# turlando/flac-py

Measured on AMD Instinct MI355X. Metric: PCM samples/sec encode-analysis, 4608-blk/16-bit mono, 1/2/4/8 MI355X, higher is better.
Workload: dtype i16 in; f64 autocorrelation/Levinson; i32 predictors; 1 GPU; 1e6 synthetic mono 4608-sample int16 blocks, -l 12 -q 5 -r 0,5; units_per_gpu=1000000, units_total=1000000, block=4608, sample_bits=16, max_lpc_order=12, qlp_precision=5, mode=reference, parallelism=dp1 (block shards), open_eighths=0, lpc_pruning=on: candidates proven to lose skipped (sign bound, partial-sum tiers)

## Files before the change

### flac-py_amd/csrc/flacmi_host.cpp

```cpp
#include <dlfcn.h>
#include <hip/hip_runtime.h>

#include <algorithm>
#include <atomic>
#include <cerrno>
#include <chrono>
#include <cmath>
#include <cstdarg>
#include <cstdio>
#include <cstdlib>
#include <cstring>
#include <map>
#include <mutex>
#include <string>
#include <vector>

#include "../../include/flacmi.h"
#include "flacmi_kernels.h"
#include "pymath.h"
#include "device_common.h"

using namespace flacmi;

static double (*volatile libm_cos)(double) = cos;
// ... 94 lines not shown
    return w;
}

struct DevBuf {
    void* p = nullptr;
    size_t bytes = 0;
};

struct flacmi_ctx {
    int device = 0;
    hipStream_t stream = nullptr;
    double* d_log2thr = nullptr;
    int32_t* d_sintab = nullptr;
    std::map<int, double*> windows;
    std::map<int, std::pair<int, int>> window_one;
    DevBuf rec, retry, h_samples, h_meta, h_params, h_residual, h_acf, h_fs, h_ls, h_recs;
    uint16_t* d_crc = nullptr;
    DevBuf scan, h_offsets, h_status, h_frames, dec, slow;
    DevBuf h_subkind;
    DevBuf h_side, h_choice;
    DevBuf idx, sd_data, sd_table, sd_meta, sd_rows, sd_pcm;
    int64_t frames_bytes = 0;
    static constexpr int kRing = 64;
    static constexpr int kMaxChunks = 8;
    hipEvent_t ev[kRing][3 + 2 * kMaxChunks] = {};
    int nchunks[kRing] = {};
    hipEvent_t lpc_done[kMaxChunks] = {};
    int ncalls = 0;
    struct EncState* enc = nullptr;
};
static void enc_free(struct EncState* es);
// ... 117 lines not shown
    if ((e = hipMemcpy(ctx->d_sintab, g_sintab.data(), sizeof(int32_t) * 4096, hipMemcpyHostToDevice)) != hipSuccess)
        return bad(e, "hipMemcpy");
    const std::vector<uint16_t> crc = crc16_tables();
    if ((e = hipMalloc(&ctx->d_crc, sizeof(uint16_t) * crc.size())) != hipSuccess) return bad(e, "hipMalloc");
    if ((e = hipMemcpy(ctx->d_crc, crc.data(), sizeof(uint16_t) * crc.size(), hipMemcpyHostToDevice)) != hipSuccess)
        return bad(e, "hipMemcpy");
    return ctx;
}

void flacmi_destroy(flacmi_ctx* ctx) {
    if (!ctx) return;
    (void)hipSetDevice(ctx->device);
    (void)hipDeviceSynchronize();
    enc_free(ctx->enc);
    for (auto& kv : ctx->windows) (void)hipFree(kv.second);
    for (DevBuf* b : {&ctx->idx, &ctx->sd_data, &ctx->sd_table, &ctx->sd_meta, &ctx->sd_rows, &ctx->sd_pcm, &ctx->slow, &ctx->dec, &ctx->rec, &ctx->retry, &ctx->h_samples, &ctx->h_meta, &ctx->h_params, &ctx->h_residual, &ctx->h_acf,
                      &ctx->h_fs, &ctx->h_ls, &ctx->h_recs, &ctx->scan, &ctx->h_offsets, &ctx->h_status,
                      &ctx->h_frames, &ctx->h_subkind, &ctx->h_side, &ctx->h_choice})
        if (b->p) (void)hipFree(b->p);
    if (ctx->d_log2thr) (void)hipFree(ctx->d_log2thr);
    if (ctx->d_sintab) (void)hipFree(ctx->d_sintab);
    if (ctx->d_crc) (void)hipFree(ctx->d_crc);
    for (auto& slot : ctx->ev)
        for (auto& ev : slot)
            if (ev) (void)hipEventDestroy(ev);
    if (ctx->stream) (void)hipStreamDestroy(ctx->stream);
    for (auto& ev : ctx->lpc_done)
        if (ev) (void)hipEventDestroy(ev);
    delete ctx;
}

// ... 143 lines not shown
}

constexpr int64_t kOverlapMinUnits = 16384;
static int overlap_mode() { return knob(kKnobOverlap); }

static int analyze_device_impl(flacmi_ctx* ctx, const flacmi_batch* b, const flacmi_params* p,
                               const flacmi_outputs* o, hipStream_t s, bool allow_overlap = true) {
    if (int rc = set_device(ctx)) return rc;
    const bool lpc = p->mode == FLACMI_MODE_REFERENCE || p->mode == FLACMI_MODE_LPC_ONLY;
    const int L = lpc ? p->max_lpc_order : 0;
    const int rec_words = FLACMI_LPC_REC_WORDS(L);
    if (lpc) {
        if (int rc = ensure_buf(ctx->rec, sizeof(int32_t) * (size_t)rec_words * (size_t)(b->n_units > 0 ? b->n_units : 1)))
            return rc;
    }
    constexpr int64_t kSubWords = 64 * 16;
    if (int rc = ensure_buf(ctx->retry, sizeof(int64_t) * (size_t)(kSubWords + 2 * b->n_units + 68))) return rc;
    struct Cls {
        int64_t unit0, count;
        int n;
    } cls[2];
    int ncls = 0;
    const int64_t nfull = b->n_units - b->n_tail_units;
    if (b->n_tail_units == 0 || b->tail_len == b->block_len) {
        cls[ncls++] = {0, b->n_units, b->block_len};
    } else {
        if (nfull > 0) cls[ncls++] = {0, nfull, b->block_len};
        cls[ncls++] = {nfull, b->n_tail_units, b->tail_len};
    }
    if (o->acf && !lpc)
// ... 23 lines not shown
                ch[nch++] = {cls[c].unit0, whole, cls[c].n};
                ch[nch++] = {cls[c].unit0 + whole, rest, cls[c].n};
                overlap = true;
                continue;
            }
        }
        int64_t k = overlap && ov > 1 ? cls[c].count / kOverlapMinUnits : 1;
        const int left = flacmi_ctx::kMaxChunks - nch - (ncls - 1 - c);
        k = k < 1 ? 1 : k > want ? want : k;
        k = k > left ? left : k;
        for (int64_t i = 0; i < k; ++i) {
            const int64_t u0 = cls[c].count * i / k, u1 = cls[c].count * (i + 1) / k;
            ch[nch++] = {cls[c].unit0 + u0, u1 - u0, cls[c].n};
        }
    }
    auto lpc_args = [&](const Chunk& k, LpcArgs& a) -> int {
        a = LpcArgs{};
        a.samples = b->samples;
        a.stride = b->unit_stride;
        a.unit0 = k.unit0;
        a.count = k.count;
        a.sample_bytes = b->sample_bytes;
        a.n = k.n;
        a.L = L;
        a.q = p->qlp_precision;
        a.lpc_sign = (p->reserved[1] & FLACMI_FLAG_LPC_SIGN) != 0;
        if (int rc = get_window(ctx, k.n, (double**)&a.window, &a.fuse_lo, &a.fuse_hi)) return rc;
        if (b->sample_bits > 26) a.fuse_lo = a.fuse_hi = 0;
        a.log2thr = ctx->d_log2thr;
        a.rec = (int32_t*)ctx->rec.p + k.unit0 * rec_words;
        a.rec_words = rec_words;
        a.acf = o->acf ? o->acf + k.unit0 * 33 : nullptr;
        return 0;
    };
    auto launch_resid_chunk = [&](const Chunk& k, hipStream_t st) -> hipError_t {
        ResidArgs a{};
        a.samples = b->samples;
        a.stride = b->unit_stride;
        a.unit0 = k.unit0;
        a.count = k.count;
        a.sample_bytes = b->sample_bytes;
        a.n = k.n;
        a.L = L;
        a.mode = p->mode;
        a.rmin = p->rice_min;
        a.rmax = p->rice_max;
        a.rec = lpc ? (const int32_t*)ctx->rec.p + k.unit0 * rec_words : nullptr;
        a.rice_order = p->mode == FLACMI_MODE_RICE_ONLY ? p->reserved[0] : 0;
        a.rec_words = rec_words;
        a.log2thr = ctx->d_log2thr;
        a.meta = o->meta + k.unit0;
        a.rice_params = o->rice_params + k.unit0 * o->params_stride;
        a.params_stride = o->params_stride;
        a.residual = (char*)o->residual + (size_t)k.unit0 * o->residual_stride * o->residual_bytes;
        a.residual_stride = o->residual_stride;
        a.fixed_sums = o->fixed_sums ? o->fixed_sums + k.unit0 * 5 : nullptr;
        a.lpc_sums = o->lpc_sums ? o->lpc_sums + k.unit0 * 32 : nullptr;
        a.stop_after = debug_stop();
        a.mfma = use_mfma();
        int64_t* const rb = (int64_t*)ctx->retry.p;
        a.retry_sub = (unsigned long long*)rb;
        a.retry_count = (unsigned long long*)(rb + kSubWords);
        a.retry_list = rb + kSubWords + 2;
        a.retry2_count = (unsigned long long*)(rb + kSubWords + 2 + b->n_units + 64);
        a.retry2_list = rb + kSubWords + 4 + b->n_units + 64;
        a.sample_bits = b->sample_bits;
        a.stream = use_stream();
        a.prune = p->mode == FLACMI_MODE_REFERENCE && !o->lpc_sums &&
                  !(p->reserved[1] & (FLACMI_FLAG_ALL_CANDIDATES | FLACMI_FLAG_LPC_SIGN)) && prune_allowed();
        a.sign_bound = !(p->reserved[1] & FLACMI_FLAG_TIERS_ONLY) && sign_bound_allowed();
        const bool wide = needs_wide(k.n, b->sample_bits, L, p->qlp_precision, p->mode);
        int path = (wide || o->residual_bytes == 8) ? 2 : (b->sample_bytes == 2 && p->qlp_precision <= 16) ? 0 : 1;
        if (path == 2 && o->residual_bytes == 4 && split_ok(b->sample_bits, L, p->qlp_precision)) path = 3;
        return launch_resid(a, path, o->residual_bytes, st);
    };
    const int slot = ctx->ncalls % flacmi_ctx::kRing;
    hipEvent_t* ev = ctx->ev[slot];
    hipStream_t side = nullptr;
    if (overlap && !allow_overlap) overlap = false;
    if (overlap) {
        if (int rc = enc_streams(ctx)) return rc;
        side = enc_side(ctx);
        if (side == s) overlap = false;
    }
    ctx->nchunks[slot] = overlap ? nch : 0;
    HIP_TRY(hipEventRecord(ev[0], s));
    if (overlap) {
        HIP_TRY(hipStreamWaitEvent(side, ev[0], 0));
// ... 1456 lines not shown
```

### flac-py_amd/csrc/flacmi_kernels.h

```cpp
#pragma once
#include <hip/hip_runtime.h>
#include <stdint.h>

#include "../../include/flacmi.h"

namespace flacmi {

constexpr int kWindowPad = 80;

struct LpcArgs {
    const void* samples;
    int64_t stride;
    int64_t unit0, count;
    int32_t sample_bytes;
    int32_t n, L, q;
    const double* window;
    const double* log2thr;
    int32_t* rec;
    int32_t rec_words;
    int32_t lpc_sign;
    double* acf;
    int32_t fuse_lo, fuse_hi;
};

struct ResidArgs {
    const void* samples;
    int64_t stride;
    int64_t unit0, count;
    int32_t sample_bytes;
    int32_t n, L, mode;
    int32_t rmin, rmax;
    int32_t rice_order;
    const int32_t* rec;
    int32_t rec_words;
    const double* log2thr;
    flacmi_unit_meta* meta;
    int32_t* rice_params;
// ... 3 lines not shown
    int64_t* fixed_sums;
    int64_t* lpc_sums;
    int32_t stop_after;
    int32_t mfma;
    unsigned long long* retry_count;
    int64_t* retry_list;
    unsigned long long* retry2_count;
    int64_t* retry2_list;
    unsigned long long* retry_sub;
    int64_t retry_sub_cap;
    int32_t sample_bits;
    int32_t stream;
    int32_t prune;
    int32_t persist;
    int32_t sign_bound;
};
#define FLACMI_STATUS_RETRY 0x7e

struct StereoChoice {
    int32_t code;
    int32_t status;
    int64_t unit[2];
};

struct FrameArgs {
    const void* samples;
    int64_t stride;
    int32_t sample_bytes;
    int32_t block_len, tail_len;
    int64_t n_units, n_tail_units;
// ... 115 lines not shown
};

ResidLaunch resid_launch_config(int n, int rmax_eff, int residual_bytes);
constexpr int kMaxFinestParts = 4096;

enum Knob { kKnobOverlap = 0, kKnobMf8Grid, kKnobStreamGeneric, kKnobDecodeGeneric, kKnobPackGeneric, kKnobDecodeLpc, kKnobCount };
int knob(Knob k);

hipError_t launch_lpc(const LpcArgs& a, hipStream_t s);
int64_t lpc_units_per_round(const LpcArgs& a);
hipError_t launch_poison_lds(hipStream_t s);
hipError_t launch_export(const int64_t* off, const int32_t* st, int64_t nf, int64_t* h_off, int32_t* h_st,
                         hipStream_t s);
hipError_t launch_lpc_from_acf(const LpcArgs& a, hipStream_t s);
hipError_t launch_resid(const ResidArgs& a, int path, int residual_bytes, hipStream_t s);
hipError_t launch_expand_records(const int32_t* rec, int32_t rec_words, int32_t L, int64_t count,
                                 int32_t* out, hipStream_t s);
hipError_t launch_synth(void* dst, int32_t sample_bytes, int32_t bits, int64_t stride,
                        int64_t first_unit, int64_t n_units, int32_t len, uint64_t seed,
                        const int32_t* sintab, int32_t open8, hipStream_t s);
hipError_t launch_stats(const flacmi_unit_meta* meta, int64_t n_units, int32_t block_len,
                        int32_t tail_len, int64_t n_tail_units, int64_t* stats, hipStream_t s);

hipError_t launch_stereo_rows(const void* lr, int32_t sample_bytes, int64_t lr_stride, int64_t n_frames,
                              int32_t block_len, int32_t tail_len, int32_t has_tail, void* mid, int64_t mid_stride,
                              int32_t* side, int64_t side_stride, hipStream_t s);
hipError_t launch_stereo_choose(const FrameArgs& a, hipStream_t s);

hipError_t launch_frame_sizes(const FrameArgs& a, int64_t* bsum, hipStream_t s);
int64_t frame_scan_blocks(int64_t n_frames);
// ... 11 lines not shown
```

### flac-py_amd/csrc/k_lpc.hip

```cpp
#include <type_traits>

#include <map>
#include <mutex>
#include <utility>

#include "device_common.h"

namespace flacmi {


template <int LMAX>
__device__ __forceinline__ void write_quant(int32_t* rec, int L, int p, const int32_t* q, int nq,
                                            int shift) {
    rec[2 + p - 1] = shift;
    int32_t* c = rec + 2 + L + (p * (p - 1)) / 2;
#pragma unroll
    for (int j = 0; j < LMAX; ++j)
        if (j < p) c[j] = j < nq ? q[j] : 0;
}

template <int LMAX>
__device__ __forceinline__ void lpc_finish(const double (&acc)[LMAX + 1], const LpcArgs& a, int32_t* __restrict__ rec) {
    const int L = a.L, q = a.q;
    const pym::PowTables PT{c_log_hdr, c_log_tab, c_exp_hdr, c_exp_tab};
    double c[LMAX + 1];
    c[0] = 1.0;
#pragma unroll
    for (int j = 1; j <= LMAX; ++j) c[j] = 0.0;
    double err = acc[0];
    int lst = ST_OK, lsite = 0, qst = ST_OK, qsite = 0;
    uint32_t negmask = 0;
    const double qmax = (double)((1LL << (q - 1)) - 1);
    const double qmin = -(double)(1LL << (q - 1));
    const uint64_t sign = a.lpc_sign ? 1ull << 63 : 0;
    static_for<LMAX>([&](auto K_) {
        constexpr int k = K_;
        if (k < L && lst == ST_OK) {
            double lam = 0.0;
#pragma unroll
            for (int j = 0; j <= k; ++j) lam = lam - c[j] * acc[k + 1 - j];
            if (err == 0.0) {
                lst = ST_ZERODIV;
                lsite = FLACMI_SITE_LEVINSON_DIV;
            } else {
                lam = lam / err;
#pragma unroll
                for (int nn = 0; nn <= (k + 1) / 2; ++nn) {
                    const double tmp = c[k + 1 - nn] + lam * c[nn];
                    c[nn] = c[nn] + lam * c[k + 1 - nn];
                    c[k + 1 - nn] = tmp;
                }
// ... 2 lines not shown
                if (pst) {
                    lst = ST_OVERFLOW;
                    lsite = FLACMI_SITE_LEVINSON_POW;
                } else {
                    err = err * (1.0 - l2);
                }
            }
            if (lst == ST_OK && qst == ST_OK) {
                const int p = k + 1;
                double cm = __builtin_fabs(c[1]);
#pragma unroll
                for (int j = 2; j <= LMAX; ++j)
                    if (j <= p && __builtin_fabs(c[j]) > cm) cm = __builtin_fabs(c[j]);
                int32_t* __restrict__ cq = rec + 2 + L + (p * (p - 1)) / 2;
                int shift = 0;
                if (!(cm > 0.0)) {
                    qst = ST_ASSERT;
                    qsite = FLACMI_SITE_QUANT_CMAX;
                } else if (__builtin_isinf(cm)) {
                    qst = ST_OVERFLOW;
                    qsite = FLACMI_SITE_QUANT_LOG2;
                } else {
                    shift = q - pym::py_floor_log2(cm, a.log2thr) - 2;
                    if (shift > 15) shift = 15;
                    if (shift < -16) {
                        qst = ST_ASSERT;
                        qsite = FLACMI_SITE_QUANT_SHIFT;
                    } else {
                        const bool neg = shift < 0;
                        const double scale = pym::as_double(((uint64_t)(1023 + (neg ? -shift : shift)) << 52) | sign);
// ... 1 lines not shown
#pragma unroll
                        for (int j = 1; j <= LMAX; ++j) {
                            if (j <= p && qst == ST_OK) {
                                e = e + c[j] * scale;
                                if (__builtin_isinf(e)) {
                                    qst = ST_OVERFLOW;
                                    qsite = FLACMI_SITE_QUANT_ROUND_INF;
                                } else if (__builtin_isnan(e)) {
                                    qst = ST_VALUE;
                                    qsite = FLACMI_SITE_QUANT_ROUND_NAN;
                                } else {
                                    const double r = __builtin_rint(e);
                                    const double qq = r < qmin ? qmin : (r > qmax ? qmax : r);
                                    e = e - qq;
                                    cq[j - 1] = (int32_t)qq;
                                }
                            }
                        }
                        if (qst == ST_OK) {
                            if (neg) {
                                negmask |= 1u << k;
                                shift = 0;
#pragma unroll
                                for (int j = 0; j < LMAX; ++j)
                                    if (j < p) cq[j] = 0;
                            }
                            rec[2 + p - 1] = shift;
                        }
                    }
                }
            }
        }
    });
    int st = lst != ST_OK ? lst : qst;
    int site = lst != ST_OK ? lsite : qsite;
    if (st == ST_OK && L == 0) {
        st = ST_VALUE;
        site = FLACMI_SITE_LPC_EMPTY;
    }
    rec[0] = st | (site << 16);
    rec[1] = (int32_t)negmask;
}

constexpr int lpc_waves(int lmax, int sample_bytes = 4) { return lmax <= 12 ? 3 : sample_bytes == 4 ? 2 : 1; }

template <int LMAX, typename SampleT, bool ACF_IN = false>
__global__ __launch_bounds__(256) __attribute__((amdgpu_waves_per_eu(lpc_waves(LMAX, (int)sizeof(SampleT))))) void k_lpc(LpcArgs a) {
    const int64_t gid = (int64_t)blockIdx.x * 256 + threadIdx.x;
    if (gid >= a.count) return;
    const int64_t u = a.unit0 + gid;
    const SampleT* __restrict__ x = (const SampleT*)a.samples + u * a.stride;
    int32_t* __restrict__ rec = a.rec + gid * a.rec_words;
    const int n = a.n, L = a.L;

    constexpr int S = ((LMAX + 1 + 7) / 8) * 8;
    double acc[LMAX + 1];
// ... 144 lines not shown
                    }
                }
            }
        }
#pragma unroll
        for (int w = 0; w < W; ++w) cur[w] = nxt[w];
    }
    }
    if (a.acf) {
        double* o = a.acf + gid * 33;
#pragma unroll
        for (int l = 0; l < 33; ++l) o[l] = (l <= LMAX && l <= L) ? acc[l < LMAX ? l : LMAX] : 0.0;
    }
    }

    lpc_finish<LMAX>(acc, a, rec);
}


template <int LMAX>
__global__ __launch_bounds__(256) __attribute__((amdgpu_waves_per_eu(LMAX <= 12 ? 4 : 1))) void k_lpc_tile(LpcArgs a) {
    __shared__ __align__(16) uint4 tiles[4 * 512];
    const int lane = threadIdx.x & 63, wid = threadIdx.x >> 6;
    const int64_t wave0 = (int64_t)blockIdx.x * 256 + wid * 64;
    if (wave0 >= a.count) return;
    const int64_t gid = wave0 + lane;
    const int n = a.n, L = a.L;
    int32_t* __restrict__ rec = a.rec + gid * a.rec_words;
    constexpr int S = ((LMAX + 1 + 7) / 8) * 8;
    static_assert(32 % S == 0, "ring length divides a half tile");
    static_assert(64 <= kWindowPad, "the last tile's window reads stay inside the window's zero pad");
// ... 86 lines not shown
    };
    int t1 = (a.fuse_lo + LMAX + 63) >> 6;
    if (a.fuse_lo + LMAX <= 0) t1 = 0;
    int t2 = min(a.fuse_hi, M) >> 6;
    if (t2 > ntile) t2 = ntile;
    if (t1 > t2) t1 = t2;
    if (ntile > 0) issue(0);
    for (int tI = 0; tI < t1; ++tI) tile_body(tI, T0{});
    for (int tI = t1; tI < t2; ++tI) tile_body(tI, T1{});
    for (int tI = t2; tI < ntile; ++tI) tile_body(tI, T0{});
    if (a.acf) {
        double* o = a.acf + gid * 33;
#pragma unroll
        for (int l = 0; l < 33; ++l) o[l] = (l <= LMAX && l <= L) ? acc[l < LMAX ? l : LMAX] : 0.0;
    }
    lpc_finish<LMAX>(acc, a, rec);
}


static bool lpc_tile_enabled() {
    static const bool on = [] {
        const char* e = getenv("FLACMI_LPC_TILE");
        return !(e && e[0] == '0');
    }();
    return on;
}

template <int LMAX>
static hipError_t launch_lpc_T(const LpcArgs& a, hipStream_t s) {
    const dim3 grid((unsigned)((a.count + 255) / 256));
    if constexpr (LMAX <= 12) {
        const int64_t full = a.count & ~(int64_t)63;
        if (a.sample_bytes == 2 && lpc_tile_enabled() && a.stride % 8 == 0 && a.stride >= 8 && full > 0) {
            LpcArgs t = a;
            t.count = full;
            hipLaunchKernelGGL((k_lpc_tile<LMAX>), dim3((unsigned)((full + 255) / 256)), dim3(256), 0, s, t);
            if (full == a.count) return hipGetLastError();
            LpcArgs r = a;
            r.unit0 += full;
            r.count = a.count - full;
            r.rec += full * a.rec_words;
            if (r.acf) r.acf += full * 33;
            hipLaunchKernelGGL((k_lpc<LMAX, int16_t>), dim3((unsigned)((r.count + 255) / 256)), dim3(256), 0, s, r);
            return hipGetLastError();
        }
    }
    if (a.sample_bytes == 2)
        hipLaunchKernelGGL((k_lpc<LMAX, int16_t>), grid, dim3(256), 0, s, a);
    else
        hipLaunchKernelGGL((k_lpc<LMAX, int32_t>), grid, dim3(256), 0, s, a);
    return hipGetLastError();
}

hipError_t launch_lpc_from_acf(const LpcArgs& a, hipStream_t s) {
    if (a.count <= 0) return hipSuccess;
    hipLaunchKernelGGL((k_lpc<32, int32_t, true>), dim3((unsigned)((a.count + 255) / 256)), dim3(256), 0, s, a);
// ... 42 lines not shown
```

### flac-py_amd/csrc/k_stream.hip

```cpp
#include <type_traits>

#include "device_common.h"

namespace flacmi {

namespace {

typedef _Float16 h8 __attribute__((ext_vector_type(8)));
typedef float f4 __attribute__((ext_vector_type(4)));
typedef _Float16 h2 __attribute__((ext_vector_type(2)));
typedef unsigned short us2 __attribute__((ext_vector_type(2)));

#ifndef FLACMI_STREAM_CPT
#define FLACMI_STREAM_CPT 5
#endif
constexpr int kSCPT = FLACMI_STREAM_CPT;
#ifndef FLACMI_RICE_DEDUP
#define FLACMI_RICE_DEDUP 1
#endif
#ifndef FLACMI_SAD16
#define FLACMI_SAD16 1
#endif
__host__ __device__ constexpr int stream_threads(int n) {
    const int nch = n / 8;
    const int nt = 64 * ((nch + 64 * kSCPT - 1) / (64 * kSCPT));
    return nt < 64 ? 64 : nt;
}
constexpr int kSHP = 16;
constexpr uint32_t kMagicBits = 0x4B400000u;
constexpr int kCoefLimit = 127;
constexpr int kRiceOrders = 8;

struct SLds {
    int xs, pk, rec, red, red2, red0, pks, total;
};

__host__ __device__ inline SLds stream_lds(int n, int nw, int tap_words, int P, int RS) {
    auto up = [](int b) { return (b + 15) & ~15; };
    auto mx = [](int x, int y) { return x > y ? x : y; };
    SLds l;
    int o = 0;
    l.xs = o;   o = up(o + 2 * (kSHP + n));
    l.pk = l.rec = o; o = up(o + mx(2 * P * RS, 4 * mx(tap_words, 1)));
    l.red = l.red2 = o; o = up(o + mx(8 * nw * 16, 8 * (nw + 1) * kRiceOrders));
    l.red0 = o; o = up(o + 4 * nw);
    l.pks = o;  o = up(o + 4 * P);
    l.total = o;
    return l;
}

__host__ __device__ constexpr int tap_table_words(int NG) { return NG > 0 ? 40 * NG + 1 : 0; }
__device__ __forceinline__ uint32_t f16_of_int(int v) {
    return (uint32_t)__builtin_bit_cast(unsigned short, (_Float16)(float)v);
}

constexpr uint32_t f16_bits(int v) {
    if (v == 0) return 0;
    const uint32_t sgn = v < 0 ? 0x8000u : 0u;
    const int m = v < 0 ? -v : v;
    int e = 0;
    while ((m >> (e + 1)) != 0) ++e;
    return sgn | (uint32_t)((e + 15) << 10) | (uint32_t)((m << (10 - e)) & 0x3ff);
}
constexpr int fixed_tap(int p, int j) {
    if (j == 0) return -1;
    if (j < 0 || j > p) return 0;
    int c = 1;
    for (int t = 0; t < j; ++t) c = c * (p - t) / (t + 1);
    return (j & 1) ? c : -c;
// ... 157 lines not shown
template <int NG, bool R05, int NFIX, bool LIST, typename Args>
__device__ __forceinline__ void stream_unit(const Args& a, const int64_t gid, unsigned char* smem) {
    const int tid = LIST ? (int)opaque((uint32_t)threadIdx.x) : (int)threadIdx.x, NT = NFIX ? stream_threads(NFIX) : (int)blockDim.x, lane = tid & 63, nw = NT >> 6;
#if FLACMI_STREAM_STAMPS
    uint64_t stamp[8];
    const uint64_t rt0 = __builtin_amdgcn_s_memrealtime();
    stamp[0] = __builtin_amdgcn_s_memtime();
#define STAMP(k) (stamp[k] = __builtin_amdgcn_s_memtime())
#else
#define STAMP(k) ((void)0)
#endif
    const int wid = __builtin_amdgcn_readfirstlane(tid >> 6);
    const int n = NFIX ? NFIX : a.n, L = NG > 0 ? (NFIX ? 4 * NG : a.L) : 0;
    const int nch = n >> 3, nblk = n >> 6;
    const int rw = NG > 0 ? (NFIX ? 2 + L + (L * (L + 1)) / 2 : a.rec_words) : 0;
    int rmax_eff = -1;
    for (int o = a.rmin; o <= a.rmax; ++o)
        if (n % (1 << o) == 0) rmax_eff = o;
    const int Pmax = 1 << rmax_eff;
    constexpr int RS = kRiceOrders;
    const SLds lay = stream_lds(n, nw, tap_table_words(NG), Pmax, RS);
    uint16_t* xs = reinterpret_cast<uint16_t*>(smem + lay.xs) + kSHP;
    int32_t* recl = reinterpret_cast<int32_t*>(smem + lay.rec);
    uint32_t* red0 = reinterpret_cast<uint32_t*>(smem + lay.red0);
    unsigned long long* red2 = reinterpret_cast<unsigned long long*>(smem + lay.red2);
    uint32_t* pks = reinterpret_cast<uint32_t*>(smem + lay.pks);
    uint16_t* pkw = reinterpret_cast<uint16_t*>(smem + lay.pk);
    flacmi_unit_meta* meta = a.meta + gid;
    MetaVals mv{};

    uint4 fixb;
    {
        const uint4* src = reinterpret_cast<const uint4*>((const int16_t*)a.samples + (a.unit0 + gid) * a.stride);
        uint4 q[kSCPT];
#pragma unroll
        for (int j = 0; j < kSCPT; ++j) {
#if FLACMI_NT_LOAD
            typedef unsigned int v4u __attribute__((ext_vector_type(4)));
            const v4u t = __builtin_nontemporal_load(reinterpret_cast<const v4u*>(src) + min(tid + j * NT, nch - 1));
            q[j] = uint4{t.x, t.y, t.z, t.w};
#else
            q[j] = src[min(tid + j * NT, nch - 1)];
#endif
        }
        fixb = reinterpret_cast<const uint4*>(kFixB.w)[lane];
        constexpr int kTW = tap_table_words(NG), kTJ = NG > 0 ? (kTW + 63) / 64 : 0;
        int32_t tv[kTJ > 0 ? kTJ : 1][2];
        if constexpr (NG > 0) {
            const int32_t* r = a.rec + gid * rw;
#pragma unroll
            for (int j = 0; j < kTJ; ++j) {
                if (j > 0 && j * NT >= kTW) break;
                const int gw = tid + j * NT, p = gw / 10 + 1, w = gw - 10 * (p - 1);
                const int pc = p < L ? p : L, base = 2 + L + (pc * (pc - 1)) / 2;
                tv[j][0] = r[w == 8 ? 1 + pc : min(max(base + 15 - 2 * w, 0), rw - 1)];
                tv[j][1] = r[min(max(base + 14 - 2 * w, 0), rw - 1)];
            }
        }
        if (tid < kSHP) xs[tid - kSHP] = 0x8000u;
        if (tid < Pmax) pks[tid] = a.stop_after == 10 ? (uint32_t)n * 40u : 0u;
#if FLACMI_SAD16
        const uint32_t k8000 = opaque(0x80008000u);
#else
        const uint32_t k8000 = opaque(0x8000u);
#endif
        uint32_t sumx = 0;
#pragma unroll
        for (int j = 0; j < kSCPT; ++j) {
            const int v = tid + j * NT;
            if (v < nch) {
                const uint4 y{q[j].x ^ 0x80008000u, q[j].y ^ 0x80008000u, q[j].z ^ 0x80008000u, q[j].w ^ 0x80008000u};
// ... 3 lines not shown
                for (int e = 0; e < 4; ++e) {
#if FLACMI_SAD16
                    sumx = __builtin_amdgcn_sad_u16(yd[e], k8000, sumx);
#else
                    sumx = sad32(yd[e] & 0xffffu, k8000, sumx);
                    sumx = sad32(yd[e] >> 16, k8000, sumx);
#endif
                }
            }
        }
        if constexpr (NG > 0) {
            uint32_t* tt = reinterpret_cast<uint32_t*>(recl);
#pragma unroll
            for (int j = 0; j < kTJ; ++j) {
                if (j > 0 && j * NT >= kTW) break;
                const int gw = tid + j * NT, p = gw / 10 + 1, w = gw - 10 * (p - 1);
                if (gw < kTW) {
                    auto tap = [&](int i, int32_t c) -> uint32_t {
                        if (p > L || i < 0 || i > p) return 0u;
                        return f16_of_int(i == 0 ? -(1 << c) : c);
                    };
                    tt[gw] = tap(16 - 2 * w, tv[j][0]) | tap(15 - 2 * w, tv[j][1]) << 16;
                }
            }
        }
        const uint32_t sx = wave_sum_u32(sumx);
        if (lane == 0) red0[wid] = sx;
    }
    STAMP(1);
    __syncthreads();
    STAMP(2);
    uint32_t negmask = 0;
    const int32_t* __restrict__ grec = NG > 0 ? a.rec + gid * rw : nullptr;
    if constexpr (NG > 0) {
        const int st = grec[0];
        if (st != 0) {
            if (wid == 0) {
                mv.status = st & 0xffff;
                mv.site = st >> 16;
                store_meta(meta, lane, mv, 0);
            }
            return;
        }
        negmask = (uint32_t)grec[1];
    }

    const bool prune = NG > 0 && a.prune && !LIST;
    unsigned long long* red64 = reinterpret_cast<unsigned long long*>(smem + lay.red);
    auto lane_total = [&]() __attribute__((always_inline)) -> uint64_t {
        uint64_t t = 0;
        int g = -1, o4l = 0;
        if (lane >= 1 && lane <= 4) {
            g = 0;
            o4l = lane - 1;
        } else if (NG > 0 && lane >= 16 && lane < 16 + 4 * NG) {
            g = 1 + ((lane - 16) >> 2);
            o4l = (lane - 16) & 3;
        }
        if (g >= 0) {
// ... 2 lines not shown
        } else if (lane == 0) {
#pragma unroll 1
            for (int w2 = 0; w2 < nw; ++w2) t += red0[w2];
        }
        return t;
    };
    uint64_t tj = 0;
    bool pruned = false;
    {
        const int col = lane & 15, kb = lane >> 4, o4 = col >> 2, rho = col & 3;
        h8 B[NG + 1];
        int shg[NG + 1];
        const uint32_t* tt = reinterpret_cast<const uint32_t*>(recl);
        const int k0 = 4 + 4 * kb - rho;
        const uint32_t alb = 16u * (uint32_t)(k0 & 1);
        bool outside = false;
#pragma unroll
        for (int g = 0; g <= NG; ++g) {
            int sh = 0;
            if (g == 0) {
                B[0] = __builtin_bit_cast(h8, fixb);
            } else {
                const int p = 4 * (g - 1) + o4 + 1, wb = 10 * (p - 1) + (k0 >> 1);
                const uint32_t w0 = tt[wb], w1 = tt[wb + 1], w2 = tt[wb + 2];
                uint32_t l0 = __builtin_amdgcn_alignbit(w1, w0, alb), l2 = __builtin_amdgcn_alignbit(w2, w1, alb);
                if constexpr (LIST) {
                    const uint32_t keep = kb == 3 ? ((rho & 1) ? 0x0000ffffu : 0xffff0000u) : 0xffffffffu;
                    l0 &= rho < 2 ? keep : 0xffffffffu;
                    l2 &= rho >= 2 ? keep : 0xffffffffu;
                }
                const h2 k256{(_Float16)256.0f, (_Float16)256.0f};
                const uint32_t h0 = __builtin_bit_cast(uint32_t, __builtin_bit_cast(h2, l0) * k256);
                const uint32_t hh = __builtin_bit_cast(uint32_t, __builtin_bit_cast(h2, l2) * k256);
                B[g] = __builtin_bit_cast(h8, uint4{h0, hh, l0, l2});
                const h2 one{(_Float16)1.0f, (_Float16)1.0f};
                float sw = __builtin_amdgcn_fdot2(__builtin_bit_cast(h2, l0 & 0x7fff7fffu), one, 0.0f, false);
                sw = __builtin_amdgcn_fdot2(__builtin_bit_cast(h2, l2 & 0x7fff7fffu), one, sw, false);
                sw += __shfl_xor(sw, 16);
                sw += __shfl_xor(sw, 32);
                outside |= rho == 0 && p <= L && sw > (float)kCoefLimit;
                const uint32_t t0 = tt[10 * (p - 1) + 8] & 0xffffu;
                sh = p <= L ? (int)((t0 >> 10) & 31u) - 15 : 0;
            }
            shg[g] = sh;
        }
        if (NG > 0 && __ballot(outside)) {
            if (tid == 0) {
                meta->status = FLACMI_STATUS_RETRY;
                if constexpr (LIST) {
                    const unsigned long long k = atomicAdd(a.retry2_count, 1ull);
                    a.retry2_list[k] = gid;
                } else {
                    const int r = (int)(gid & 63);
                    const unsigned long long k = atomicAdd(a.retry_sub + 16 * r, 1ull);
                    a.retry_list[r * a.retry_sub_cap + (int64_t)k] = gid;
                }
            }
            return;
        }
        if (a.stop_after == 1) return;
        auto start_of = [&](int g) __attribute__((always_inline)) -> int {
            const int p = 4 * (g > 0 ? g - 1 : 0) + o4 + 1;
            return (g > 0 && ((negmask >> (p - 1)) & 1)) ? 0 : p;
        };
        const uint32_t mbv = opaque_s(kMagicBits);
        const f4 C{12582912.0f, 12582912.0f, 12582912.0f, 12582912.0f};
        const int eoff = 4 * (lane & 15) - 12 + 4 * kb;
        uint32_t acc[NG + 1];
#pragma unroll
        for (int g = 0; g <= NG; ++g) acc[g] = 0;
        auto ld = [&](int blk) __attribute__((always_inline)) {
            return *reinterpret_cast<const uint2*>(xs + 64 * blk + eoff);
        };
// ... 556 lines not shown
        const uint32_t base = r > 0 ? (uint32_t)__builtin_amdgcn_readlane((int)incl, r - 1) : 0u;
        stream_unit<NG, R05, NFIX, true>(*pa, pa->retry_list[r * pa->retry_sub_cap + (k - base)], smem);
        __syncthreads();
    }
}

hipError_t launch_resid_retry_l8(const ResidArgs& a, hipStream_t s);
hipError_t launch_resid_retry_l12(const ResidArgs& a, hipStream_t s);

bool stream_shape_ok(const ResidArgs& a, int path, int residual_bytes) {
    if (!a.stream || path != 0 || residual_bytes != 4 || a.sample_bytes != 2 || !a.mfma || !a.retry_list || !a.retry_count ||
        !a.retry2_list || !a.retry2_count || !a.retry_sub)
        return false;
    const bool ref = a.mode == FLACMI_MODE_REFERENCE && a.L >= 1 && a.L <= 12;
    if (!ref && a.mode != FLACMI_MODE_FIXED_ONLY) return false;
    if (a.n % 64 != 0 || a.n < 64 || a.n > 8 * kSCPT * 256) return false;
    int rmax_eff = -1;
    for (int o = a.rmin; o <= a.rmax; ++o)
        if (a.n % (1 << o) == 0) rmax_eff = o;
    if (rmax_eff < 0 || (1 << rmax_eff) > 32 || ((a.n >> rmax_eff) & 7) != 0) return false;
    return true;
}

static unsigned stream_list_grid(int64_t count) {
    int dev = 0, ncu = 0;
    if (hipGetDevice(&dev) != hipSuccess || hipDeviceGetAttribute(&ncu, hipDeviceAttributeMultiprocessorCount, dev) != hipSuccess ||
        ncu <= 0)
        ncu = 256;
    const int64_t g = 16 * (int64_t)ncu;
    return (unsigned)(count < g ? count : g);
// ... 60 lines not shown
```

Before: 417.6 billion samples/s.

## Emit pre-packed f16 tap rows from LPC kernel for stream residual kernel

The LPC kernel now writes, per block, a 128-word row holding f16-packed quantized taps, shifts, negmask, status and precomputed coefficient-bound flags, and it stages parked words through LDS so the global stores are coalesced. The stream residual kernel loads this row directly instead of gathering from the triangular rec layout, converting to f16 and running a fdot2/shuffle reduction to decide retries. This moves per-block work from the residual kernel into LPC finish. In exchange it adds an extra 512-byte-per-unit buffer and more register and LDS pressure in the LPC kernel.

```diff
diff --git a/flac-py_amd/csrc/flacmi_host.cpp b/flac-py_amd/csrc/flacmi_host.cpp
--- a/flac-py_amd/csrc/flacmi_host.cpp
+++ b/flac-py_amd/csrc/flacmi_host.cpp
@@ -132,7 +132,7 @@
     int32_t* d_sintab = nullptr;
     std::map<int, double*> windows;
     std::map<int, std::pair<int, int>> window_one;
-    DevBuf rec, retry, h_samples, h_meta, h_params, h_residual, h_acf, h_fs, h_ls, h_recs;
+    DevBuf rec, taps, retry, h_samples, h_meta, h_params, h_residual, h_acf, h_fs, h_ls, h_recs;
     uint16_t* d_crc = nullptr;
     DevBuf scan, h_offsets, h_status, h_frames, dec, slow;
     DevBuf h_subkind;
@@ -280,7 +280,7 @@
     (void)hipDeviceSynchronize();
     enc_free(ctx->enc);
     for (auto& kv : ctx->windows) (void)hipFree(kv.second);
-    for (DevBuf* b : {&ctx->idx, &ctx->sd_data, &ctx->sd_table, &ctx->sd_meta, &ctx->sd_rows, &ctx->sd_pcm, &ctx->slow, &ctx->dec, &ctx->rec, &ctx->retry, &ctx->h_samples, &ctx->h_meta, &ctx->h_params, &ctx->h_residual, &ctx->h_acf,
+    for (DevBuf* b : {&ctx->idx, &ctx->sd_data, &ctx->sd_table, &ctx->sd_meta, &ctx->sd_rows, &ctx->sd_pcm, &ctx->slow, &ctx->dec, &ctx->rec, &ctx->taps, &ctx->retry, &ctx->h_samples, &ctx->h_meta, &ctx->h_params, &ctx->h_residual, &ctx->h_acf,
                       &ctx->h_fs, &ctx->h_ls, &ctx->h_recs, &ctx->scan, &ctx->h_offsets, &ctx->h_status,
                       &ctx->h_frames, &ctx->h_subkind, &ctx->h_side, &ctx->h_choice})
         if (b->p) (void)hipFree(b->p);
@@ -454,6 +454,11 @@
         if (int rc = ensure_buf(ctx->rec, sizeof(int32_t) * (size_t)rec_words * (size_t)(b->n_units > 0 ? b->n_units : 1)))
             return rc;
     }
+    const bool tap_rows = p->mode == FLACMI_MODE_REFERENCE && L >= 1 && L <= 12 && b->sample_bytes == 2 && o->residual_bytes == 4;
+    if (tap_rows) {
+        if (int rc = ensure_buf(ctx->taps, sizeof(uint32_t) * (size_t)kTapRowWords * (size_t)(b->n_units > 0 ? b->n_units : 1)))
+            return rc;
+    }
     constexpr int64_t kSubWords = 64 * 16;
     if (int rc = ensure_buf(ctx->retry, sizeof(int64_t) * (size_t)(kSubWords + 2 * b->n_units + 68))) return rc;
     struct Cls {
@@ -507,27 +512,8 @@
             ch[nch++] = {cls[c].unit0 + u0, u1 - u0, cls[c].n};
         }
     }
-    auto lpc_args = [&](const Chunk& k, LpcArgs& a) -> int {
-        a = LpcArgs{};
-        a.samples = b->samples;
-        a.stride = b->unit_stride;
-        a.unit0 = k.unit0;
-        a.count = k.count;
-        a.sample_bytes = b->sample_bytes;
-        a.n = k.n;
-        a.L = L;
-        a.q = p->qlp_precision;
-        a.lpc_sign = (p->reserved[1] & FLACMI_FLAG_LPC_SIGN) != 0;
-        if (int rc = get_window(ctx, k.n, (double**)&a.window, &a.fuse_lo, &a.fuse_hi)) return rc;
-        if (b->sample_bits > 26) a.fuse_lo = a.fuse_hi = 0;
-        a.log2thr = ctx->d_log2thr;
-        a.rec = (int32_t*)ctx->rec.p + k.unit0 * rec_words;
-        a.rec_words = rec_words;
-        a.acf = o->acf ? o->acf + k.unit0 * 33 : nullptr;
-        return 0;
-    };
-    auto launch_resid_chunk = [&](const Chunk& k, hipStream_t st) -> hipError_t {
-        ResidArgs a{};
+    auto resid_args = [&](const Chunk& k, ResidArgs& a) -> int {
+        a = ResidArgs{};
         a.samples = b->samples;
         a.stride = b->unit_stride;
         a.unit0 = k.unit0;
@@ -541,6 +527,7 @@
         a.rec = lpc ? (const int32_t*)ctx->rec.p + k.unit0 * rec_words : nullptr;
         a.rice_order = p->mode == FLACMI_MODE_RICE_ONLY ? p->reserved[0] : 0;
         a.rec_words = rec_words;
+        a.taps = tap_rows ? (const uint32_t*)ctx->taps.p + k.unit0 * kTapRowWords : nullptr;
         a.log2thr = ctx->d_log2thr;
         a.meta = o->meta + k.unit0;
         a.rice_params = o->rice_params + k.unit0 * o->params_stride;
@@ -565,6 +552,33 @@
         const bool wide = needs_wide(k.n, b->sample_bits, L, p->qlp_precision, p->mode);
         int path = (wide || o->residual_bytes == 8) ? 2 : (b->sample_bytes == 2 && p->qlp_precision <= 16) ? 0 : 1;
         if (path == 2 && o->residual_bytes == 4 && split_ok(b->sample_bits, L, p->qlp_precision)) path = 3;
+        return path;
+    };
+    auto lpc_args = [&](const Chunk& k, LpcArgs& a) -> int {
+        a = LpcArgs{};
+        a.samples = b->samples;
+        a.stride = b->unit_stride;
+        a.unit0 = k.unit0;
+        a.count = k.count;
+        a.sample_bytes = b->sample_bytes;
+        a.n = k.n;
+        a.L = L;
+        a.q = p->qlp_precision;
+        a.lpc_sign = (p->reserved[1] & FLACMI_FLAG_LPC_SIGN) != 0;
+        if (int rc = get_window(ctx, k.n, (double**)&a.window, &a.fuse_lo, &a.fuse_hi)) return rc;
+        if (b->sample_bits > 26) a.fuse_lo = a.fuse_hi = 0;
+        a.log2thr = ctx->d_log2thr;
+        a.rec = (int32_t*)ctx->rec.p + k.unit0 * rec_words;
+        a.rec_words = rec_words;
+        a.acf = o->acf ? o->acf + k.unit0 * 33 : nullptr;
+        ResidArgs r;
+        const int path = resid_args(k, r);
+        a.taps = tap_rows && stream_shape_ok(r, path, o->residual_bytes) ? (uint32_t*)ctx->taps.p + k.unit0 * kTapRowWords : nullptr;
+        return 0;
+    };
+    auto launch_resid_chunk = [&](const Chunk& k, hipStream_t st) -> hipError_t {
+        ResidArgs a;
+        const int path = resid_args(k, a);
         return launch_resid(a, path, o->residual_bytes, st);
     };
     const int slot = ctx->ncalls % flacmi_ctx::kRing;
diff --git a/flac-py_amd/csrc/flacmi_kernels.h b/flac-py_amd/csrc/flacmi_kernels.h
--- a/flac-py_amd/csrc/flacmi_kernels.h
+++ b/flac-py_amd/csrc/flacmi_kernels.h
@@ -7,6 +7,10 @@
 namespace flacmi {
 
 constexpr int kWindowPad = 80;
+
+constexpr int kTapRowWords = 128;
+constexpr int kTapTrail = 120;
+constexpr int kTapCoefLimit = 127;
 
 struct LpcArgs {
     const void* samples;
@@ -21,6 +25,7 @@
     int32_t lpc_sign;
     double* acf;
     int32_t fuse_lo, fuse_hi;
+    uint32_t* taps;
 };
 
 struct ResidArgs {
@@ -54,6 +59,7 @@
     int32_t prune;
     int32_t persist;
     int32_t sign_bound;
+    const uint32_t* taps;
 };
 #define FLACMI_STATUS_RETRY 0x7e
 
@@ -199,6 +205,7 @@
                          hipStream_t s);
 hipError_t launch_lpc_from_acf(const LpcArgs& a, hipStream_t s);
 hipError_t launch_resid(const ResidArgs& a, int path, int residual_bytes, hipStream_t s);
+bool stream_shape_ok(const ResidArgs& a, int path, int residual_bytes);
 hipError_t launch_expand_records(const int32_t* rec, int32_t rec_words, int32_t L, int64_t count,
                                  int32_t* out, hipStream_t s);
 hipError_t launch_synth(void* dst, int32_t sample_bytes, int32_t bits, int64_t stride,
diff --git a/flac-py_amd/csrc/k_lpc.hip b/flac-py_amd/csrc/k_lpc.hip
--- a/flac-py_amd/csrc/k_lpc.hip
+++ b/flac-py_amd/csrc/k_lpc.hip
@@ -19,9 +19,55 @@
         if (j < p) c[j] = j < nq ? q[j] : 0;
 }
 
+__device__ __forceinline__ uint32_t f16_of_int(int v) {
+    return (uint32_t)__builtin_bit_cast(unsigned short, (_Float16)(float)v);
+}
+
+constexpr int tap_off(int k) {
+    int o = 0;
+    for (int p = 1; p <= k; ++p) o += (p + 1) / 2;
+    return o;
+}
+constexpr int kParkOrders = 10, kTapParked = tap_off(kParkOrders), kParkSegs = 10 * kParkOrders / 4;
 template <int LMAX>
-__device__ __forceinline__ void lpc_finish(const double (&acc)[LMAX + 1], const LpcArgs& a, int32_t* __restrict__ rec) {
+struct TapRegs {
+    uint32_t w[tap_off(LMAX) > 0 ? tap_off(LMAX) : 1];
+    uint32_t status, negmask, shw[2], flag_t, flag_c;
+    template <int I>
+    __device__ __forceinline__ uint32_t word(int L) const {
+        if constexpr (I < kTapTrail) {
+            constexpr int k = I / 10, wi = I % 10, m = 8 - wi;
+            if constexpr (k >= LMAX) return 0u;
+            else if constexpr (wi == 8)
+                return k < L ? 0x8000u | (((shw[k / 8] >> (4 * (k % 8))) & 15u) + 15u) << 10 : 0u;
+            else if constexpr (m >= 1 && m <= (k + 2) / 2) return w[tap_off(k) + m - 1];
+            else return 0u;
+        } else {
+            constexpr int t = I - kTapTrail;
+            return t == 1 ? status : t == 2 ? negmask : t == 3 ? shw[0] : t == 4 ? shw[1] : t == 5 ? flag_t : t == 6 ? flag_c : 0u;
+        }
+    }
+    static constexpr bool live(int I) {
+        const int k = I / 10, wi = I % 10, m = 8 - wi;
+        return I < kTapTrail && k < LMAX && (wi == 8 || (m >= 1 && m <= (k + 2) / 2));
+    }
+    template <int S>
+    __device__ __forceinline__ uint4 seg(int L) const {
+        return uint4{word<4 * S>(L), word<4 * S + 1>(L), word<4 * S + 2>(L), word<4 * S + 3>(L)};
+    }
+};
+
+template <int LMAX, bool ROW, bool PARK = false>
+__device__ __forceinline__ void lpc_finish(const double (&acc)[LMAX + 1], const LpcArgs& a, int32_t* __restrict__ rec,
+                                           TapRegs<ROW ? LMAX : 0>& row, uint32_t* park = nullptr,
+                                           uint32_t* __restrict__ grow = nullptr) {
     const int L = a.L, q = a.q;
+    uint32_t shw[2] = {0u, 0u}, flag_t = 0, flag_c = 0;
+    if constexpr (ROW) {
+#pragma unroll
+        for (int i = 0; i < tap_off(LMAX); ++i)
+            if (!PARK || i >= kTapParked) row.w[i] = 0u;
+    }
     const pym::PowTables PT{c_log_hdr, c_log_tab, c_exp_hdr, c_exp_tab};
     double c[LMAX + 1];
     c[0] = 1.0;
@@ -35,6 +81,12 @@
     const uint64_t sign = a.lpc_sign ? 1ull << 63 : 0;
     static_for<LMAX>([&](auto K_) {
         constexpr int k = K_;
+        if constexpr (ROW && PARK && k >= kParkOrders) {
+            if (grow && k >= L) {
+#pragma unroll
+                for (int w = 0; w < 5; ++w) reinterpret_cast<uint2*>(grow + 10 * k)[w] = uint2{0u, 0u};
+            }
+        }
         if (k < L && lst == ST_OK) {
             double lam = 0.0;
 #pragma unroll
@@ -67,6 +119,8 @@
                     if (j <= p && __builtin_fabs(c[j]) > cm) cm = __builtin_fabs(c[j]);
                 int32_t* __restrict__ cq = rec + 2 + L + (p * (p - 1)) / 2;
                 int shift = 0;
+                uint32_t tw[6] = {0u, 0u, 0u, 0u, 0u, 0u};
+                int sabs = 0;
                 if (!(cm > 0.0)) {
                     qst = ST_ASSERT;
                     qsite = FLACMI_SITE_QUANT_CMAX;
@@ -98,6 +152,11 @@
                                     const double qq = r < qmin ? qmin : (r > qmax ? qmax : r);
                                     e = e - qq;
                                     cq[j - 1] = (int32_t)qq;
+                                    if constexpr (ROW) {
+                                        const int qi = (int32_t)qq;
+                                        sabs += qi < 0 ? -qi : qi;
+                                        tw[(16 - j) / 2 - 2] |= f16_of_int(qi) << (16 * (j & 1));
+                                    }
                                 }
                             }
                         }
@@ -108,8 +167,32 @@
 #pragma unroll
                                 for (int j = 0; j < LMAX; ++j)
                                     if (j < p) cq[j] = 0;
+                                sabs = 0;
+#pragma unroll
+                                for (int w = 0; w < 6; ++w) tw[w] = 0u;
                             }
                             rec[2 + p - 1] = shift;
+                            if constexpr (ROW && PARK && k >= kParkOrders) {
+                                if (grow) {
+                                    uint2* const rp = reinterpret_cast<uint2*>(grow + 10 * k);
+                                    rp[0] = uint2{0u, 0u};
+                                    rp[1] = uint2{tw[0], tw[1]};
+                                    rp[2] = uint2{tw[2], tw[3]};
+                                    rp[3] = uint2{tw[4], tw[5]};
+                                    rp[4] = uint2{0x8000u | (uint32_t)(shift + 15) << 10, 0u};
+                                }
+                            } else if constexpr (ROW) {
+#pragma unroll
+                                for (int m = 1; m <= (p + 1) / 2; ++m) {
+                                    if (PARK && tap_off(k) + m - 1 < kTapParked) park[64 * (tap_off(k) + m - 1)] = tw[6 - m];
+                                    else row.w[tap_off(k) + m - 1] = tw[6 - m];
+                                }
+                            }
+                            if constexpr (ROW) {
+                                shw[k / 8] |= (uint32_t)shift << (4 * (k % 8));
+                                flag_t |= (sabs + (1 << shift) > kTapCoefLimit ? 1u : 0u) << k;
+                                flag_c |= (sabs > kTapCoefLimit ? 1u : 0u) << k;
+                            }
                         }
                     }
                 }
@@ -124,6 +207,12 @@
     }
     rec[0] = st | (site << 16);
     rec[1] = (int32_t)negmask;
+    if constexpr (ROW) {
+        row.status = (uint32_t)(st | (site << 16));
+        row.negmask = negmask;
+        row.shw[0] = shw[0], row.shw[1] = shw[1];
+        row.flag_t = flag_t, row.flag_c = flag_c;
+    }
 }
 
 constexpr int lpc_waves(int lmax, int sample_bytes = 4) { return lmax <= 12 ? 3 : sample_bytes == 4 ? 2 : 1; }
@@ -298,7 +387,18 @@
     }
     }
 
-    lpc_finish<LMAX>(acc, a, rec);
+    constexpr bool ROW = LMAX <= 12 && sizeof(SampleT) == 2 && !ACF_IN;
+    TapRegs<ROW ? LMAX : 0> row;
+    lpc_finish<LMAX, ROW>(acc, a, rec, row);
+    if constexpr (ROW) {
+        if (a.taps) {
+            uint4* const o = reinterpret_cast<uint4*>(a.taps + gid * kTapRowWords);
+            static_for<kTapRowWords / 4>([&](auto S_) {
+                constexpr int S = S_;
+                o[S] = row.template seg<S>(L);
+            });
+        }
+    }
 }
 
 
@@ -415,7 +515,44 @@
 #pragma unroll
         for (int l = 0; l < 33; ++l) o[l] = (l <= LMAX && l <= L) ? acc[l < LMAX ? l : LMAX] : 0.0;
     }
-    lpc_finish<LMAX>(acc, a, rec);
+    constexpr bool ROW = LMAX <= 12;
+    TapRegs<ROW ? LMAX : 0> row;
+    uint32_t* const park = ROW ? reinterpret_cast<uint32_t*>(tile) + lane : nullptr;
+    if constexpr (ROW) {
+#pragma unroll
+        for (int i = 0; i < kTapParked && i < tap_off(LMAX); ++i) park[64 * i] = 0u;
+    }
+    uint32_t* const grow = (ROW && a.taps) ? a.taps + gid * kTapRowWords : nullptr;
+    lpc_finish<LMAX, ROW, ROW>(acc, a, rec, row, park, grow);
+    if constexpr (ROW) {
+#pragma unroll
+        for (int i = 0; i < kTapParked && i < tap_off(LMAX); ++i) row.w[i] = park[64 * i];
+        asm volatile("s_waitcnt lgkmcnt(0)" ::: "memory");
+        if (a.taps) {
+            reinterpret_cast<uint4*>(grow)[kTapTrail / 4] = row.template seg<kTapTrail / 4>(L);
+            reinterpret_cast<uint4*>(grow)[kTapTrail / 4 + 1] = row.template seg<kTapTrail / 4 + 1>(L);
+            uint4* const gout = reinterpret_cast<uint4*>(a.taps + wave0 * kTapRowWords);
+            const int r16 = lane & 15;
+#pragma unroll
+            for (int t = 0; t < 8; ++t) tile[64 * t + lane] = uint4{0u, 0u, 0u, 0u};
+            uint32_t* const img = reinterpret_cast<uint32_t*>(tile) + 128 * r16;
+#pragma unroll 1
+            for (int qd = 0; qd < 4; ++qd) {
+                if ((lane >> 4) == qd)
+                    static_for<4 * kParkSegs>([&](auto I_) {
+                        constexpr int I = I_;
+                        if constexpr (TapRegs<LMAX>::live(I)) img[4 * ((I / 4 + r16) & 31) + I % 4] = row.template word<I>(L);
+                    });
+                asm volatile("s_waitcnt lgkmcnt(0)" ::: "memory");
+#pragma unroll
+                for (int t = 0; t < (16 * kParkSegs + 63) / 64; ++t) {
+                    const int o = 64 * t + lane, r = o / kParkSegs, i = o - kParkSegs * r;
+                    if (o < 16 * kParkSegs) gout[32 * (16 * qd + r) + i] = tile[32 * r + ((i + r) & 31)];
+                }
+                asm volatile("s_waitcnt lgkmcnt(0)" ::: "memory");
+            }
+        }
+    }
 }
 
 
@@ -441,6 +578,7 @@
             r.unit0 += full;
             r.count = a.count - full;
             r.rec += full * a.rec_words;
+            if (r.taps) r.taps += full * kTapRowWords;
             if (r.acf) r.acf += full * 33;
             hipLaunchKernelGGL((k_lpc<LMAX, int16_t>), dim3((unsigned)((r.count + 255) / 256)), dim3(256), 0, s, r);
             return hipGetLastError();
diff --git a/flac-py_amd/csrc/k_stream.hip b/flac-py_amd/csrc/k_stream.hip
--- a/flac-py_amd/csrc/k_stream.hip
+++ b/flac-py_amd/csrc/k_stream.hip
@@ -28,7 +28,8 @@
 }
 constexpr int kSHP = 16;
 constexpr uint32_t kMagicBits = 0x4B400000u;
-constexpr int kCoefLimit = 127;
+static_assert((kTapCoefLimit + 1) * 33023 > (1 << 22) && kTapCoefLimit * 33023 < (1 << 22),
+              "(sum|c| + 2^shift) * 33023 < 2^22: the bound k_lpc's row flags decide");
 constexpr int kRiceOrders = 8;
 
 struct SLds {
@@ -50,9 +51,7 @@
 }
 
 __host__ __device__ constexpr int tap_table_words(int NG) { return NG > 0 ? 40 * NG + 1 : 0; }
-__device__ __forceinline__ uint32_t f16_of_int(int v) {
-    return (uint32_t)__builtin_bit_cast(unsigned short, (_Float16)(float)v);
-}
+static_assert(tap_table_words(3) <= kTapTrail + 1, "the table ends at the tap row's zero word in front of its trailing words");
 
 constexpr uint32_t f16_bits(int v) {
     if (v == 0) return 0;
@@ -240,9 +239,10 @@
     const int n = NFIX ? NFIX : a.n, L = NG > 0 ? (NFIX ? 4 * NG : a.L) : 0;
     const int nch = n >> 3, nblk = n >> 6;
     const int rw = NG > 0 ? (NFIX ? 2 + L + (L * (L + 1)) / 2 : a.rec_words) : 0;
-    int rmax_eff = -1;
-    for (int o = a.rmin; o <= a.rmax; ++o)
-        if (n % (1 << o) == 0) rmax_eff = o;
+    int rmax_eff = R05 ? 5 : -1;
+    if constexpr (!R05)
+        for (int o = a.rmin; o <= a.rmax; ++o)
+            if (n % (1 << o) == 0) rmax_eff = o;
     const int Pmax = 1 << rmax_eff;
     constexpr int RS = kRiceOrders;
     const SLds lay = stream_lds(n, nw, tap_table_words(NG), Pmax, RS);
@@ -271,16 +271,13 @@
         }
         fixb = reinterpret_cast<const uint4*>(kFixB.w)[lane];
         constexpr int kTW = tap_table_words(NG), kTJ = NG > 0 ? (kTW + 63) / 64 : 0;
-        int32_t tv[kTJ > 0 ? kTJ : 1][2];
+        uint32_t tv[kTJ > 0 ? kTJ : 1];
         if constexpr (NG > 0) {
-            const int32_t* r = a.rec + gid * rw;
+            const uint32_t* r = a.taps + gid * kTapRowWords;
 #pragma unroll
             for (int j = 0; j < kTJ; ++j) {
                 if (j > 0 && j * NT >= kTW) break;
-                const int gw = tid + j * NT, p = gw / 10 + 1, w = gw - 10 * (p - 1);
-                const int pc = p < L ? p : L, base = 2 + L + (pc * (pc - 1)) / 2;
-                tv[j][0] = r[w == 8 ? 1 + pc : min(max(base + 15 - 2 * w, 0), rw - 1)];
-                tv[j][1] = r[min(max(base + 14 - 2 * w, 0), rw - 1)];
+                tv[j] = r[min(tid + j * NT, kTW - 1)];
             }
         }
         if (tid < kSHP) xs[tid - kSHP] = 0x8000u;
@@ -314,14 +311,8 @@
 #pragma unroll
             for (int j = 0; j < kTJ; ++j) {
                 if (j > 0 && j * NT >= kTW) break;
-                const int gw = tid + j * NT, p = gw / 10 + 1, w = gw - 10 * (p - 1);
-                if (gw < kTW) {
-                    auto tap = [&](int i, int32_t c) -> uint32_t {
-                        if (p > L || i < 0 || i > p) return 0u;
-                        return f16_of_int(i == 0 ? -(1 << c) : c);
-                    };
-                    tt[gw] = tap(16 - 2 * w, tv[j][0]) | tap(15 - 2 * w, tv[j][1]) << 16;
-                }
+                const int gw = tid + j * NT;
+                if (gw < kTW) tt[gw] = tv[j];
             }
         }
         const uint32_t sx = wave_sum_u32(sumx);
@@ -330,10 +321,11 @@
     STAMP(1);
     __syncthreads();
     STAMP(2);
-    uint32_t negmask = 0;
+    uint32_t negmask = 0, shw0 = 0, shw1 = 0;
     const int32_t* __restrict__ grec = NG > 0 ? a.rec + gid * rw : nullptr;
     if constexpr (NG > 0) {
-        const int st = grec[0];
+        const uint32_t* __restrict__ tr = a.taps + gid * kTapRowWords + kTapTrail;
+        const int st = (int)tr[1];
         if (st != 0) {
             if (wid == 0) {
                 mv.status = st & 0xffff;
@@ -342,7 +334,23 @@
             }
             return;
         }
-        negmask = (uint32_t)grec[1];
+        negmask = tr[2];
+        shw0 = tr[3];
+        shw1 = tr[4];
+        if (tr[LIST ? 6 : 5] != 0) {
+            if (tid == 0) {
+                meta->status = FLACMI_STATUS_RETRY;
+                if constexpr (LIST) {
+                    const unsigned long long k = atomicAdd(a.retry2_count, 1ull);
+                    a.retry2_list[k] = gid;
+                } else {
+                    const int r = (int)(gid & 63);
+                    const unsigned long long k = atomicAdd(a.retry_sub + 16 * r, 1ull);
+                    a.retry_list[r * a.retry_sub_cap + (int64_t)k] = gid;
+                }
+            }
+            return;
+        }
     }
 
     const bool prune = NG > 0 && a.prune && !LIST;
@@ -375,7 +383,6 @@
         const uint32_t* tt = reinterpret_cast<const uint32_t*>(recl);
         const int k0 = 4 + 4 * kb - rho;
         const uint32_t alb = 16u * (uint32_t)(k0 & 1);
-        bool outside = false;
 #pragma unroll
         for (int g = 0; g <= NG; ++g) {
             int sh = 0;
@@ -394,30 +401,9 @@
                 const uint32_t h0 = __builtin_bit_cast(uint32_t, __builtin_bit_cast(h2, l0) * k256);
                 const uint32_t hh = __builtin_bit_cast(uint32_t, __builtin_bit_cast(h2, l2) * k256);
                 B[g] = __builtin_bit_cast(h8, uint4{h0, hh, l0, l2});
-                const h2 one{(_Float16)1.0f, (_Float16)1.0f};
-                float sw = __builtin_amdgcn_fdot2(__builtin_bit_cast(h2, l0 & 0x7fff7fffu), one, 0.0f, false);
-                sw = __builtin_amdgcn_fdot2(__builtin_bit_cast(h2, l2 & 0x7fff7fffu), one, sw, false);
-                sw += __shfl_xor(sw, 16);
-                sw += __shfl_xor(sw, 32);
-                outside |= rho == 0 && p <= L && sw > (float)kCoefLimit;
-                const uint32_t t0 = tt[10 * (p - 1) + 8] & 0xffffu;
-                sh = p <= L ? (int)((t0 >> 10) & 31u) - 15 : 0;
+                sh = (int)(((g <= 2 ? shw0 : shw1) >> (4 * o4 + 16 * ((g - 1) & 1))) & 15u);
             }
             shg[g] = sh;
-        }
-        if (NG > 0 && __ballot(outside)) {
-            if (tid == 0) {
-                meta->status = FLACMI_STATUS_RETRY;
-                if constexpr (LIST) {
-                    const unsigned long long k = atomicAdd(a.retry2_count, 1ull);
-                    a.retry2_list[k] = gid;
-                } else {
-                    const int r = (int)(gid & 63);
-                    const unsigned long long k = atomicAdd(a.retry_sub + 16 * r, 1ull);
-                    a.retry_list[r * a.retry_sub_cap + (int64_t)k] = gid;
-                }
-            }
-            return;
         }
         if (a.stop_after == 1) return;
         auto start_of = [&](int g) __attribute__((always_inline)) -> int {
@@ -1004,6 +990,7 @@
         return false;
     const bool ref = a.mode == FLACMI_MODE_REFERENCE && a.L >= 1 && a.L <= 12;
     if (!ref && a.mode != FLACMI_MODE_FIXED_ONLY) return false;
+    if (ref && !a.taps) return false;
     if (a.n % 64 != 0 || a.n < 64 || a.n > 8 * kSCPT * 256) return false;
     int rmax_eff = -1;
     for (int o = a.rmin; o <= a.rmax; ++o)
```

Result: no change. 417.1 billion samples/s (median of 2 runs) (-0.1%).
